# engyasin/EKF-MonoSLAM_for_3D-reconstruction

Measured on AMD Instinct MI355X. Metric: EKF updates/sec at N features (state dim 14+6N), higher is better.
Workload: dtype f32 (state, covariance, every accumulation and every other contraction in fp32; the products of the covariance downdate as 3 x bf16 splits of the fp32 operands, six bf16 products per fp32 product: the dropped terms are <= 2^-24 |a||b| in the worst case (2^-28 on average) -- the size of the fp32 prod; 1 GPU; N=1000 inverse-depth features, n=6014, M=N measured per frame, fp32, 1xMI355X (BASELINE configs[2]); features=1000, state_dim=6014, measured_per_frame=1000, camera=conf_kinect.cfg/scale2, frames_per_map=3000, maps=1

## Files before the change

ekf-monoslam_for_3d-reconstruction_amd/csrc/ekf_capi.hip:

```cpp
#include <hip/hip_runtime.h>

#include <algorithm>
#include <array>
#include <climits>
#include <cmath>
#include <cstdint>
#include <cstdio>
#include <cstdlib>
#include <cstring>
#include <map>
#include <mutex>
#include <string>
#include <type_traits>
#include <vector>

#include "../../include/ekf_monoslam.h"
#include "ekf_buffers.hpp"
#include "ekf_feature_table.hpp"
#include "ekf_dense.hpp"
#include "ekf_image.hpp"
#include "ekf_features.hpp"
#include "ekf_syrk6.hpp"
#include "ekf_chain.hpp"
#include "ekf_small.hpp"
// ... 15 lines not shown
#include "ekf_mesh_texture.hpp"
#include "ekf_mesh_raster.hpp"

namespace ekf {

static thread_local std::string g_create_error;

enum KernelId : int {
  KID_PREDICT_CAMERA = 0,
  KID_PROPAGATE_STRIPS,
  KID_PROPAGATE_STREAMING,
  KID_MEASURE,
  KID_INNOVATION,
  KID_SIGMA_HT,
  KID_INNOVATION_COV,
  KID_CHOL_DIAG,
  KID_CHOL_PANEL,
  KID_CHOL_TRAILING,
  KID_STATE_UPDATE,
  KID_DOWNDATE,
  KID_SOLVE,
  KID_NORMALIZE,
  KID_ADD_FEATURE,
  KID_COMPACT,
  KID_MISC,
  KID_WUPDATE,
  KID_GATHER_H,
  KID_GATHER_S,
  KID_GATHER_V,
  KID_GATHER_SIGMA,
  KID_SEED_MASK,
  KID_SEED_RESPONSE,
  KID_SEED_CANDIDATES,
  KID_SEED_SELECT,
  KID_FRAME_UPLOAD,
  KID_FRAME_INGEST,
  KID_FRAME_RECTIFY,
  KID_COUNT
};

static const char* kKernelNames[KID_COUNT] = {
    "predict_camera",  "propagate_strips", "propagate_streaming", "measure",
    "innovation",      "sigma_ht",         "innovation_cov",      "chol_diag",
    "chol_panel",      "chol_trailing",    "state_update",        "downdate_syrk",
    "solve_trmm",      "normalize_quat",  "add_feature",      "compact_transform",   "misc",
    "w_update", "allgather_h", "allgather_s", "allgather_v", "allgather_sigma",
    "seed_mask", "seed_response", "seed_candidates", "seed_select", "frame_upload", "frame_ingest", "frame_rectify"};

static const char* kLaunchNames[EKF_LAUNCH_KINDS] = {
    "downdate_bf16x6", "downdate_f32", "downdate_f32_fused_wu", "downdate_f32_half_tail", "downdate_f32_t64",
    "row_rider", "row_gemv", "row_tile_gemm", "w_update_gemm", "w_recompute",
    "chain_step_launches", "chain_persistent", "solve", "solve_two_groups", "update_oneblock", "update_allinone",
    "chain_trail_diag", "split_image", "state_update_tail", "update_onelaunch", "chain_dist_gather", "chain_step_fused",
    "downdate_mirror_bounds", "solve_poll_chain"};

static inline int round_up(int v, int a) { return (v + a - 1) / a * a; }

struct MaskedStreamPool {
  struct Entry { int device, num_cus, reserved; hipStream_t st; };
  std::mutex mu;
  std::vector<Entry> idle;
  bool hooked = false;
  static void at_exit();
  hipStream_t take(int device, int num_cus, int reserved) {
    std::lock_guard<std::mutex> lk(mu);
    for (size_t i = 0; i < idle.size(); ++i)
      if (idle[i].device == device && idle[i].num_cus == num_cus && idle[i].reserved == reserved) {
        hipStream_t st = idle[i].st;
        idle.erase(idle.begin() + i);
        return st;
      }
    return nullptr;
  }
  void give(int device, int num_cus, int reserved, hipStream_t st) {
    std::lock_guard<std::mutex> lk(mu);
    idle.push_back({device, num_cus, reserved, st});
    if (!hooked) { hooked = true; atexit(&MaskedStreamPool::at_exit); }
  }
};
static MaskedStreamPool g_masked_streams;
void MaskedStreamPool::at_exit() {
  std::lock_guard<std::mutex> lk(g_masked_streams.mu);
  for (const Entry& e : g_masked_streams.idle) {
    if (hipSetDevice(e.device) != hipSuccess) continue;
    (void)hipStreamSynchronize(e.st);
    (void)hipStreamDestroy(e.st);
  }
  g_masked_streams.idle.clear();
}

struct FilterBase {
  std::string err;
  bool diag_synced = false;
  virtual ~FilterBase() {}
  virtual int set_dt(double) = 0;
  virtual double get_dt() const = 0;
  virtual int set_stream(void*) = 0;
  virtual int set_option(int, int) = 0;
  virtual int synchronize() = 0;
  virtual int add_feature(double, double) = 0;
  virtual int remove_features(const int*, int) = 0;
  virtual int predict(const void*, const void*, int) = 0;
  virtual int measure() = 0;
  virtual int motion_jacobian(void*, void*) = 0;
  virtual int get_predictions(void*, unsigned char*, unsigned char*, void*, void*, void*) = 0;
  virtual int update(const void*, const int*, int, int, bool) = 0;
  virtual int innovation_covariance(const int*, int, int, void*) = 0;
// ... 114 lines not shown
  DevBuf<T> d_K;
  int last_m = 0, last_m_pad = 0, last_n = 0;
  bool have_meas = false;
  bool have_sd = false;
  bool have_update = false;
  int opt_streaming = 0, opt_mfma = 1;
  hipStream_t stream = nullptr;
  bool own_stream = false;
  hipStream_t stream_b = nullptr;
  hipEvent_t ev_chain[8] = {}, ev_solve[8] = {}, ev_b = nullptr, ev_wu = nullptr;
  hipStream_t stream_g = nullptr;
  bool stream_b_masked = false;
  int stream_b_reserved = 0;
  hipEvent_t ev_gath[8] = {}, ev_g = nullptr;
  int solve64_off = 0, solve6464_off = 0, tri64_off = 0, tri64_count = 0;
  int tri6_off = 0;
  int trih_off = 0, trih_count = 0;
  int opt_split_tail = -1;
  double opt_feature_noise = 0.0;
  int opt_split_bf16 = 1;
  DevBuf<s6_u32x4> d_Vimg;
  hipError_t ensure_vimg() { return d_Vimg.reserve((size_t)(n_pad + 128) * ldy * 6 / sizeof(s6_u32x4)); }
  int last_nchunks = 1, last_cend[8] = {};
  DevBuf<unsigned char> d_frame;
  int frame_w = 0, frame_h = 0;
  bool have_frame = false, have_blur = false;
  DevBuf<unsigned char> d_raw;
  int raw_w = 0, raw_h = 0, raw_c = 0;
  bool have_raw = false;
  RectScratch rect;
  DevBuf<int4> d_ingest_tab;
  int ingest_tab_w = 0, ingest_tab_h = 0;
  DevBuf<unsigned char> d_patch[2], d_mpatch[2];
  int cur_patch = 0;
  DevBuf<T> d_hb, d_zm;
  DevBuf<unsigned char> d_found;
  DevBuf<float> d_score;
  DevBuf<int> d_keep;
  int opt_panel_direct = 1;
  int opt_chain_fused_diag = 1;
  int opt_small_onelaunch = 1;
  int opt_step_fused = 1;
  struct StepPlan { std::vector<int> off, cnt; } sfp;
  WorkList sf_lists{{0}, {}};
  DevBuf<unsigned long long> d_small_stamps;
  unsigned small_gate_total = 0;
  int opt_su_tail = 1;
  int opt_syrk_mirror_skip = 1;
  int opt_solve_poll_chain = 1;
  int opt_fuse_split = 1;
  int opt_chain_defer = 1;
  int td_min_blocks = 24;
  int td_max_blocks = 1 << 30;
  WorkList td_blocks;
  std::vector<int> td_off, td_cnt;
  int opt_syrk_stag_half = 0, opt_syrk_stag_mod4 = 2;
  int opt_solve_s2 = 1;
  bool want_solve_s2(int width, int npad_live) const {
    return kIsF32 && opt_mfma && opt_solve_s2 && (opt_solve_s2 > 1 || (width / 128) * (npad_live / 64) <= 2 * num_cus);
  }
  int opt_fused = 1;
  int opt_solve_one_per_cu = 1;
  int opt_wrecompute = 1;
  int opt_row_gemv = 1;
  int opt_fuse_wu = 1;
  int env_chunks[8] = {}, env_nchunks = 0;
  int opt_pipeline = -1;
  WorkList tilemap{{0, 0}, {}};
  int tri_count = 0, solve_off = 0;
  int w_zeroed_n = -1;
  DevBuf<int> d_counters;
  int num_cus = 256, reserved_cus = 32;
  LaunchProfiler<KID_COUNT> prof{KID_DOWNDATE, KID_PROPAGATE_STREAMING};

  static constexpr bool kIsF32 = sizeof(T) == 4;
  int NB() const { return (kIsF32 && opt_mfma) ? 128 : 64; }

  ~Filter() override {
    const bool dbg = getenv("EKF_DEBUG_DTOR") != nullptr;
    auto mark = [&](const char* what) { if (dbg) { fprintf(stderr, "[ekf dtor %p] %s\n", (void*)this, what); fflush(stderr); } };
    hipSetDevice(device);
    mark("sync main stream");
    if (stream) hipStreamSynchronize(stream);
    mark("sync side streams");
    if (stream_b) hipStreamSynchronize(stream_b);
    if (stream_g) hipStreamSynchronize(stream_g);
    mark("events");
    prof.release();
    in_ring.release();
    mark("streams");
    if (own_stream && stream) hipStreamDestroy(stream);
    mark("stream b");
    const char* pool_env = getenv("EKF_MASKED_STREAM_POOL");
    if (stream_b && stream_b_masked && !(pool_env && atoi(pool_env) == 0)) g_masked_streams.give(device, num_cus, stream_b_reserved, stream_b);
    else if (stream_b) hipStreamDestroy(stream_b);
    mark("stream g");
    if (stream_g) hipStreamDestroy(stream_g);
    mark("last events");
    for (auto e : ev_gath) if (e) hipEventDestroy(e);
    if (ev_g) hipEventDestroy(ev_g);
    for (auto e : ev_chain) if (e) hipEventDestroy(e);
    for (auto e : ev_solve) if (e) hipEventDestroy(e);
    if (ev_b) hipEventDestroy(ev_b);
    if (ev_wu) hipEventDestroy(ev_wu);
    mark("done");
  }
// ... 71 lines not shown
    HIPCHK(d_tmp.reserve(64));
    HIPCHK(d_counters.reserve(kResetInts + kMirrorRowsInts));
    HIPCHK(hipMemset(d_counters, 0, (kResetInts + kMirrorRowsInts) * sizeof(int)));
    {
      hipDeviceProp_t prop;
      HIPCHK(hipGetDeviceProperties(&prop, device));
      num_cus = prop.multiProcessorCount > 0 ? prop.multiProcessorCount : 256;
    }
    {
      reserved_cus = std::min(32, num_cus / 4);
      if (const char* e = getenv("EKF_RESERVED_CUS")) reserved_cus = std::max(1, std::min(num_cus / 2, atoi(e)));
      std::vector<uint32_t> mask((num_cus + 31) / 32, 0xffffffffu);
      for (int i = 0; i < reserved_cus; ++i) mask[i / 32] &= ~(1u << (i % 32));
      stream_b = g_masked_streams.take(device, num_cus, reserved_cus);
      stream_b_masked = stream_b != nullptr;
      if (!stream_b) {
        if (hipExtStreamCreateWithCUMask(&stream_b, (uint32_t)mask.size(), mask.data()) == hipSuccess) {
          stream_b_masked = true;
        } else {
          (void)hipGetLastError();
          stream_b = nullptr;
          reserved_cus = 0;
          HIPCHK(hipStreamCreateWithFlags(&stream_b, hipStreamNonBlocking));
        }
      }
      stream_b_reserved = reserved_cus;

      if (const char* e = getenv("EKF_FUSE_WU")) opt_fuse_wu = atoi(e);
      if (const char* e = getenv("EKF_ROW_GEMV")) opt_row_gemv = atoi(e) ? 1 : 0;
      if (const char* e = getenv("EKF_SOLVE_ONE_PER_CU")) opt_solve_one_per_cu = atoi(e) ? 1 : 0;
      if (const char* e = getenv("EKF_W_RECOMPUTE")) opt_wrecompute = atoi(e) ? 1 : 0;
      if (const char* e = getenv("EKF_SOLVE_S2")) opt_solve_s2 = atoi(e);
      if (const char* e = getenv("EKF_FUSED_LAUNCHES")) opt_fused = atoi(e) ? 1 : 0;
      if (const char* e = getenv("EKF_PANEL_DIRECT")) opt_panel_direct = atoi(e);
      if (const char* e = getenv("EKF_SYRK_STAGGER")) {
        opt_syrk_stag_half = atoi(e);
        if (const char* c = strchr(e, ',')) opt_syrk_stag_mod4 = atoi(c + 1);
      }
      if (const char* e = getenv("EKF_CHAIN_FUSED_DIAG")) opt_chain_fused_diag = atoi(e) ? 1 : 0;
      if (const char* e = getenv("EKF_FUSE_SPLIT")) opt_fuse_split = atoi(e) ? 1 : 0;
      if (const char* e = getenv("EKF_SU_TAIL")) opt_su_tail = atoi(e) ? 1 : 0;
      if (const char* e = getenv("EKF_SYRK_MIRROR_SKIP")) opt_syrk_mirror_skip = atoi(e) ? 1 : 0;
      if (const char* e = getenv("EKF_SOLVE_POLL_CHAIN")) opt_solve_poll_chain = std::max(0, std::min(2, atoi(e)));
      if (const char* e = getenv("EKF_SMALL_ONELAUNCH")) opt_small_onelaunch = atoi(e) ? 1 : 0;
      if (const char* e = getenv("EKF_STEP_FUSED")) opt_step_fused = atoi(e) ? 1 : 0;
      if (const char* e = getenv("EKF_SHARD_DIST_CHAIN")) opt_shard_dist_chain = atoi(e) ? 1 : 0;
      if (const char* e = getenv("EKF_SHARD_DIST_MIN_BLOCKS")) shard_dist_min_blocks = std::max(2, atoi(e));
      if (const char* e = getenv("EKF_SMALL_STAMPS")) {
        if (atoi(e)) { HIPCHK(d_small_stamps.reserve(16)); HIPCHK(hipMemset(d_small_stamps, 0, 16 * sizeof(unsigned long long))); }
      }
      if (const char* e = getenv("EKF_CHAIN_DEFER")) opt_chain_defer = atoi(e) ? 1 : 0;
      if (const char* e = getenv("EKF_TD_MIN_BLOCKS")) td_min_blocks = std::max(1, atoi(e));
      if (const char* e = getenv("EKF_TD_MAX_BLOCKS")) td_max_blocks = std::max(1, atoi(e));
      if (const char* e = getenv("EKF_SPLIT_TAIL")) opt_split_tail = atoi(e);
      if (const char* e = getenv("EKF_SPLIT_BF16")) opt_split_bf16 = atoi(e) ? 1 : 0;
      if (const char* e = getenv("EKF_CHUNKS")) {
        for (const char* q = e; *q && env_nchunks < 8;) {
          env_chunks[env_nchunks++] = atoi(q);
          while (*q && *q != ',') ++q;
          if (*q == ',') ++q;
        }
      }
    }
    std::vector<T> mu0(camera_dim, T(0));
    mu0[3] = T(0.0); mu0[4] = T(0.0); mu0[5] = T(-0.707106781); mu0[6] = T(0.707106781);
    if (camera_dim == 14) mu0[13] = T(1);
    n = camera_dim;
    N = 0;
    HIPCHK(hipMemcpyAsync(d_mu[0], mu0.data(), camera_dim * sizeof(T), hipMemcpyHostToDevice, stream));
    std::vector<T> S0((size_t)camera_dim * camera_dim, T(0));
    for (int i = 0; i < camera_dim; ++i) S0[(size_t)i * camera_dim + i] = T(0.0000000004);
    if (camera_dim == 14) S0[13 * 14 + 13] = T(0.09);
    const T sv2 = T(0.0004) * T(0.0004);
    for (int i = 7; i < 13; ++i) S0[(size_t)i * camera_dim + i] = sv2;
    HIPCHK(hipMemcpy2DAsync(d_S[0], (size_t)ld * sizeof(T), S0.data(), camera_dim * sizeof(T),
                            camera_dim * sizeof(T), camera_dim, hipMemcpyHostToDevice, stream));
    HIPCHK(hipStreamSynchronize(stream));
    extent[0] = n; extent[1] = 0;
    HIPCHK(hipFuncSetAttribute(reinterpret_cast<const void*>(&k_chol_diag<T, 64>),
                               hipFuncAttributeMaxDynamicSharedMemorySize, diag_lds(64)));
    if constexpr (kIsF32) {
      HIPCHK(hipFuncSetAttribute(reinterpret_cast<const void*>(&k_trail_diag),
                                 hipFuncAttributeMaxDynamicSharedMemorySize, (int)kChainLds));
    }
    return EKF_OK;
  }
  static int diag_lds(int nb) { return 2 * nb * (nb + 1) * (int)sizeof(T); }

  T* S() { return d_S[cur]; }
  T* mu() { return d_mu[cur_mu]; }

  int sync_layout() {
    if (!layout_dirty) return EKF_OK;
    if (N > 0) {
      HIPCHK(hipMemcpyAsync(d_pos, ft.columns().pos.data(), N * sizeof(int), hipMemcpyHostToDevice, stream));
      HIPCHK(hipMemcpyAsync(d_coding, ft.columns().coding.data(), N * sizeof(int), hipMemcpyHostToDevice, stream));
      HIPCHK(hipStreamSynchronize(stream));
    }
    layout_dirty = false;
    return EKF_OK;
  }

  InputRing in_ring;
  PinnedBuf<char> h_pred;
  PinnedBuf<unsigned char> h_ransac;
  static constexpr size_t kRansacMaskBytes = 65536;
// ... 745 lines not shown
    HIPCHK(hipStreamSynchronize(stream));
    if (h) memcpy(h, ph, (size_t)N * 2 * sizeof(T));
    for (int i = 0; i < N; ++i) { if (vis) vis[i] = pfl[i] & 1; if (rem) rem[i] = (pfl[i] >> 1) & 1; }
    if (s2) {
      T* o = static_cast<T*>(s2);
      const T* sd = psd;
      for (int i = 0; i < N; ++i) { o[4 * i] = sd[4 * i]; o[4 * i + 1] = sd[4 * i + 2]; o[4 * i + 2] = sd[4 * i + 1]; o[4 * i + 3] = sd[4 * i + 3]; }
    }
    if (hc) { T* o = static_cast<T*>(hc); for (int i = 0; i < N; ++i) for (int a = 0; a < 2; ++a) for (int c = 0; c < 7; ++c) o[14 * i + c * 2 + a] = vhc[14 * i + a * 7 + c]; }
    if (hf) { T* o = static_cast<T*>(hf); for (int i = 0; i < N; ++i) for (int a = 0; a < 2; ++a) for (int c = 0; c < 6; ++c) o[12 * i + c * 2 + a] = vhf[12 * i + a * 6 + c]; }
    return EKF_OK;
  }

  struct GemmCall {
    const T* A = nullptr; int lda = 0;
    const T* B = nullptr; int ldb = 0;
    T* C = nullptr; int ldc = 0;
    int rows = 0, cols = 0, K = 0;
    T alpha = T(1), beta = T(0);
    int tri = TRI_ALL, row_off = 0, col_off = 0, ktri = KTRI_FULL, ktile_off = 0;
    int zrow = 0, zcol_end = 0;
    const int* tile_list = nullptr; int ntiles = 0;
    int* counter = nullptr;
    void* img = nullptr; int img_nkc = 0, img_c0 = 0;
    bool two_groups = false;
    bool one_per_cu = false;
    const unsigned* chain_word = nullptr; unsigned chain_epoch = 0;
    hipStream_t st = nullptr;
  };
  struct Rows { int r0, count; };
  struct UpdatePlan {
    int M = 0, plane = 0;
    int nb = 0, tile = 0, m = 0, m_pad = 0, npad_live = 0, nsteps = 0;
    int nchunks = 1, cend[8] = {};
    ChunkTab tab{};
    int strip_rows = 0;
    int ntr = 0, ntc = 0;
    bool oneblock = false, allinone = false, onelaunch = false;
    int small_rc = 0, small_nchunk = 0, small_nt64 = 0;
    bool recompute = false;
    int r0 = 0, r1 = 0, p0 = 0, prows = 0;
    Rows ranges[3] = {};
    bool sym_panel = false, shard_split = false;
    int c0(int g) const { return (g ? cend[g - 1] : 0) * nb; }
    int c1(int g) const { return cend[g] * nb; }
  };
  struct UpdateCtx {
    const T* z;
    const int* midx;
    int* counters;
    int counter_next = 0;
    bool step_fused = false;
    int diag_ahead = -1;
    struct { int step = -1, c0 = 0, c1 = 0; } pending;
    bool row_pending = false;
    bool queue_room(int ints = 8) const { return counter_next + ints <= kQueueCounters; }
    int* take_queue() {
      if (!queue_room()) return nullptr;
      counter_next += 8;
      return counters + counter_next - 8;
    }
  };

  template <int ROLE, bool BT, int TM = 128, int TN = 128>
  void gemm(const GemmCall& c) {
    GemmArgs g{};
    g.A = c.A; g.lda = c.lda; g.B = c.B; g.ldb = c.ldb; g.C = c.C; g.ldc = c.ldc;
    g.K = c.K; g.alpha = double(c.alpha); g.beta = double(c.beta);
    g.tri = c.tri; g.row_off = c.row_off; g.col_off = c.col_off; g.ktri = c.ktri; g.ktile_off = c.ktile_off;
    g.zrow = c.zrow; g.zcol_end = c.zcol_end;
    g.stagger = (ROLE == ROLE_DOWNDATE) ? 1 : 0;
    g.img = c.img; g.img_nkc = c.img_nkc; g.img_c0 = c.img_c0;
    g.chain_word = c.chain_word; g.chain_epoch = c.chain_epoch; g.status = d_status;
    hipStream_t st = c.st ? c.st : stream;
    const bool mf = kIsF32 && opt_mfma;
    dim3 grid(c.cols / (mf ? TN : 64), c.rows / (mf ? TM : 64));
    if (c.tile_list && c.counter) {
      g.tile_map = c.tile_list;
      g.ntiles = c.ntiles;
      g.counter = c.counter;
      const bool side = (st == stream_b);
      int wgs = 2 * (side ? (num_cus - reserved_cus) : num_cus);
      if (ROLE == ROLE_SOLVE && c.one_per_cu) wgs = num_cus;
      grid = dim3(std::min(c.ntiles, wgs), 1);
    }
    if constexpr (kIsF32) {
      if (opt_mfma) {
        if constexpr (ROLE == ROLE_SOLVE) {
          ++launch_cnt[c.two_groups ? EKF_LAUNCH_SOLVE_TWO_GROUPS : EKF_LAUNCH_SOLVE];
          if (c.two_groups) {
            k_gemm_mfma<ROLE, BT, TM, TN, true><<<grid, 512, 0, st>>>(g);
            return;
          }
        }
        k_gemm_mfma<ROLE, BT, TM, TN><<<grid, 256, 0, st>>>(g);
        return;
      }
    }
    if constexpr (!kIsF32) {
      if (opt_mfma) {
        k_gemm_mfma_f64<ROLE, BT><<<grid, 256, 0, st>>>(g);
        return;
      }
    }
    k_gemm_valu<T, ROLE, BT><<<grid, 256, 0, st>>>(g);
  }
// ... 174 lines not shown
        constexpr int KB = 8;
        dim3 grid((m_pad + 255) / 256, std::max(1, (M + KB - 1) / KB) + (m_pad - 2 * M + 7) / 8);
        k_innovation_cov<T, KB><<<grid, 256, 0, stream>>>(d_W, ldy, d_Hc, d_Hf, d_pos, d_coding, ip, M, plane,
                                                        T(sigma_pixel_2), T(0.00001), d_Y, m_pad, 0, M, zid, N, ct, strip_rows);
      }
    }
    HIPCHK(hipGetLastError());
    if (m_out) *m_out = m;
    if (m_pad_out) *m_pad_out = m_pad;
    return EKF_OK;
  }

  bool trail_diag_ok() const {
    return kIsF32 && opt_mfma && opt_chain_fused_diag && (size_t)2 * ldy * ldy * sizeof(T) < ((size_t)1 << 31);
  }
  int ensure_trail_diag_lists(int nblk, int nchunks, const int* cend) {
    std::vector<int> key = {nblk, nchunks};
    key.insert(key.end(), cend, cend + nchunks);
    if (td_blocks.current(key)) return EKF_OK;
    std::vector<int> all;
    td_off.assign(nblk, 0);
    td_cnt.assign(nblk, 0);
    for (int g = 0; g < nchunks; ++g) {
      const int s0 = g ? cend[g - 1] : 0, s1 = cend[g];
      for (int j = s0; j < s1; ++j) {
        td_off[j] = (int)all.size();
        for (int K = j + 1; K < nblk; ++K) {
          for (int I = K; I < nblk; ++I) {
            if (I == j + 1) continue;
            all.push_back(I); all.push_back(K);
          }
          if (K < s1)
            for (int t = 0; t <= j - s0; ++t) { all.push_back(nblk + t); all.push_back(K); }
        }
        td_cnt[j] = ((int)all.size() - td_off[j]) / 2;
      }
    }
    HIPCHK(hipStreamSynchronize(stream));
    if (stream_b) HIPCHK(hipStreamSynchronize(stream_b));
    HIPCHK(td_blocks.upload(key, all, 2));
    return EKF_OK;
  }
  bool launch_trail_diag(UpdateCtx& ux, int step, int m, hipStream_t sc_) {
    if constexpr (kIsF32) {
      const int td_nblk = td_blocks.first();
      if (!trail_diag_ok() || NB() != 128 || td_nblk == 0 || step + 1 >= td_nblk || td_cnt[step] < td_min_blocks ||
          td_cnt[step] > td_max_blocks)
        return false;
      TrailDiagArgs a{};
      a.Y = d_Y; a.ldy = ldy; a.y_bytes = (unsigned)((size_t)2 * ldy * ldy * sizeof(T));
      a.Dinv = d_Dinv; a.dinv_bytes = (unsigned)((size_t)(ldy / 64) * 128 * 128 * sizeof(T));
      a.status = d_status; a.m = m; a.j = step;
      a.blocks = td_blocks.d + td_off[step]; a.nblocks = td_cnt[step]; a.do_diag = 1;
      Scope sc(this, KID_CHOL_TRAILING, sc_);
      ++launch_cnt[EKF_LAUNCH_CHAIN_TRAIL_DIAG];
      k_trail_diag<<<a.nblocks + 1, 1024, kChainLds, sc_>>>(a);
      ux.diag_ahead = step + 1;
      return true;
    }
    return false;
  }

  int ensure_step_fused_lists(int nblk) {
    const std::vector<int> key = {nblk};
    if (sf_lists.current(key)) return EKF_OK;
    std::vector<int> all;
    sfp.off.assign(nblk, 0);
    sfp.cnt.assign(nblk, 0);
    const int s0 = 0, s1 = nblk;
    for (int j = 0; j < nblk; ++j) {
      sfp.off[j] = (int)all.size();
      const int first = 2 * (j + 1);
      for (int r = first; r < 2 * nblk; ++r)
        for (int c = first; c <= r; ++c) { all.push_back(r); all.push_back(c); all.push_back(SF_TILE | (c == r ? SF_WRITE_PANEL : 0)); }
      for (int r = 2 * nblk; r < 2 * nblk + 2 * (j + 1 - s0); ++r) {
        if (first < 2 * s1) {
          for (int c = first; c < 2 * s1; ++c) { all.push_back(r); all.push_back(c); all.push_back(SF_TILE | (c == first ? SF_WRITE_PANEL : 0)); }
        } else {
          all.push_back(r); all.push_back(r); all.push_back(SF_WRITE_PANEL);
        }
      }
      sfp.cnt[j] = ((int)all.size() - sfp.off[j]) / 3;
      all[sfp.off[j] + 2] |= SF_WRITE_DIAG;
    }
    HIPCHK(hipStreamSynchronize(stream));
    HIPCHK(sf_lists.upload(key, all));
    return EKF_OK;
  }
  bool launch_step_fused(const UpdateCtx& ux, int step, int m, hipStream_t sc_) {
    if constexpr (kIsF32) {
      if (!ux.step_fused || step >= sf_lists.first() || sfp.cnt[step] > num_cus / 2 || sc_ != stream) return false;
      StepFusedArgs a{};
      a.Y = d_Y; a.ldy = ldy; a.Dj = d_Dinv + (size_t)step * 128 * 128; a.status = d_status; a.m = m; a.j = step;
      a.wl = sf_lists.d + sfp.off[step]; a.nwg = sfp.cnt[step];
      a.gate = reinterpret_cast<unsigned*>(d_status + 9);
      small_gate_total += (unsigned)a.nwg;
      a.gate_target = small_gate_total;
      Scope sc(this, KID_CHOL_TRAILING, sc_);
      ++launch_cnt[EKF_LAUNCH_CHAIN_STEP_FUSED];
      k_chain_step_fused<<<a.nwg, 1024, 0, sc_>>>(a);
      return true;
    }
    return false;
  }
  void chain_trailing(UpdateCtx& ux, int step, int c0, int c1, int m, int m_pad, hipStream_t sc_, bool allow_fused) {
    const int nb = NB();
    T* Y = d_Y;
    const int j = step * nb, r0 = j + nb;
    const int vrows = m_pad - c0, tcols = m_pad - r0;
// ... 407 lines not shown
        std::vector<int> hidx((size_t)std::max(M, 0));
        if (M > 0) {
          HIPCHK(hipMemcpyAsync(hidx.data(), idx, (size_t)M * sizeof(int), hipMemcpyDeviceToHost, stream));
          HIPCHK(hipStreamSynchronize(stream));
        }
        return shard_update(z, hidx.data(), M, plane);
      }
      if (M > 0 && z) HIPCHK(hipMemcpyAsync(d_z, z, (size_t)2 * M * sizeof(T), hipMemcpyHostToDevice, stream));
      return shard_update(d_z, idx, M, plane);
    }
    if (M < 0 || M > N) FAIL(EKF_ERR_ARG, "M out of range");
    if (M == 0 && !plane) return EKF_OK;
    if (!have_meas) FAIL(EKF_ERR_STATE, "ekf_update needs the h/H of ekf_predict or ekf_measure");
    if (M > 0 && (!z || !idx)) FAIL(EKF_ERR_ARG, "z / indices are NULL");
    if (!on_device) { int rcl = check_list(idx, M, true); if (rcl) return rcl; }
    UpdateCtx ux{d_z, d_midx, d_counters};
    if (M > 0) {
      if (on_device) {
        ux.z = static_cast<const T*>(z);
        ux.midx = idx;
      } else {
        int rcs = stage_inputs(z, idx, M);
        if (rcs) return rcs;
        sh_list.clear();
      }
    }
    const UpdatePlan p = plan_update(M, plane);
    int rc = p.onelaunch ? launch_update_small(p, ux)
                         : build_innovation(ux.z, ux.midx, M, plane, true, nullptr, nullptr, &p.tab, p.strip_rows);
    if (rc) return rc;
    rc = ensure_tilemap(p.npad_live / p.tile, p.ntr, p.ntc);
    if (rc) return rc;
    rc = prepare_chain(p, ux, false);
    if (rc) return rc;
    const int nchunks = p.nchunks, m_pad = p.m_pad;
    bool b_inflight = false;
    for (int gi = 0; gi < (p.onelaunch ? 0 : nchunks); ++gi) {
      const int c0 = p.c0(gi), c1 = p.c1(gi);
      chain_steps(ux, gi ? p.cend[gi - 1] : 0, p.cend[gi], c0, c1, p.m, m_pad, stream, p.oneblock,
                  opt_chain_defer && gi + 1 < nchunks);
      const bool overlap = chunk_overlaps(p, gi);
      hipStream_t ss = overlap ? stream_b : stream;
      if (!overlap && b_inflight) {
        if (p.recompute) {
          HIPCHK(hipEventRecord(ev_b, stream_b));
          HIPCHK(hipStreamWaitEvent(stream, ev_b, 0));
          b_inflight = false;
        } else {
          HIPCHK(hipStreamWaitEvent(stream, ev_wu, 0));
        }
      }
      if (overlap) {
        b_inflight = true;
        if (solve_polls_chain(p, gi)) {
          if constexpr (kIsF32)
            k_publish_epoch<<<1, 64, 0, stream>>>(reinterpret_cast<unsigned*>(d_counters + kChainEpochWord), (unsigned)gi + 1);
        } else {
          HIPCHK(hipEventRecord(ev_chain[gi], stream));
          HIPCHK(hipStreamWaitEvent(stream_b, ev_chain[gi], 0));
        }
      }
      bool vimg_done = false;
      rc = solve_chunk(p, gi, ux, ss, &vimg_done);
      if (rc) return rc;
      const bool fuse = chunk_fuses(p, gi, ux);
      wupdate_chunk(p, gi, ux, ss);
      if (overlap && c1 < m_pad && !fuse && !p.recompute) HIPCHK(hipEventRecord(ev_wu, stream_b));
      if (!overlap && b_inflight) {
        HIPCHK(hipEventRecord(ev_b, stream_b));
        HIPCHK(hipStreamWaitEvent(stream, ev_b, 0));
        b_inflight = false;
      }
      if (!overlap && nchunks > 1 && !chunk_su_tail(p, gi, ux)) {
        HIPCHK(hipEventRecord(ev_chain[gi], stream));
        HIPCHK(hipStreamWaitEvent(stream_b, ev_chain[gi], 0));
        launch_state_update(m_pad, stream_b);
        b_inflight = true;
      }
      rc = downdate_chunk(p, gi, ux, ss, vimg_done);
      if (rc) return rc;
      if (fuse && !p.recompute) HIPCHK(hipEventRecord(ev_wu, stream_b));
      if (p.recompute && gi + 1 < nchunks) {
        launch_w_recompute(c1, p.c1(gi + 1), m_pad, ux.midx, M, plane, ss, n);
      }
    }
    if (b_inflight) {
      HIPCHK(hipEventRecord(ev_b, stream_b));
      HIPCHK(hipStreamWaitEvent(stream, ev_b, 0));
    }
    return finish_update(p, nchunks == 1 && !p.oneblock, !p.allinone);
  }

  int innovation_covariance(const int* idx, int M, int plane, void* out) override {
    HIPCHK(hipSetDevice(device));
    if (M < 0 || M > N) FAIL(EKF_ERR_ARG, "M out of range");
    if (!have_meas) FAIL(EKF_ERR_STATE, "ekf_innovation_covariance needs ekf_predict / ekf_measure first");
    const int mm = 2 * M + (plane ? 3 : 0);
    if (mm == 0) return EKF_OK;
    int rc = check_list(idx, M, sh_on);
    if (rc) return rc;
    if (M > 0) HIPCHK(hipMemcpyAsync(d_midx, idx, (size_t)M * sizeof(int), hipMemcpyHostToDevice, stream));
    sh_list.clear();
    int m = 0, m_pad = 0;
    if (sh_on) {
      rc = shard_build_ws(idx, M, plane, nullptr, &m, &m_pad);
    } else {
// ... 4266 lines not shown
```

ekf-monoslam_for_3d-reconstruction_amd/csrc/ekf_chain.hpp:

```cpp
#pragma once
#include "ekf_dense.hpp"

namespace ekf {

constexpr unsigned kChainPimg = 75776;
constexpr unsigned kChainLds = 141568;

namespace chain {
typedef float f4 __attribute__((ext_vector_type(4)));
typedef __amdgpu_buffer_rsrc_t rsrc_t;

__device__ __forceinline__ f4 ld16(rsrc_t r, unsigned byte_off) {
  return __builtin_bit_cast(f4, __builtin_amdgcn_raw_buffer_load_b128(r, (int)byte_off, 0, 0));
}
__device__ __forceinline__ float ld4(rsrc_t r, unsigned byte_off) {
  return __builtin_bit_cast(float, __builtin_amdgcn_raw_buffer_load_b32(r, (int)byte_off, 0, 0));
}
__device__ __forceinline__ void st4(rsrc_t r, unsigned byte_off, float v) {
  __builtin_amdgcn_raw_buffer_store_b32(__builtin_bit_cast(unsigned, v), r, (int)byte_off, 0, 0);
}

__device__ __attribute__((noinline)) void trail(rsrc_t ry, unsigned ldy, int j, int I, int K, int only, f32x4* lds_all, int tid,
                                                int lane, int wave) {
  constexpr int NQ = 8, TS = 64, STAGE = NQ * (TS + TS), BK = 32, NG = BK / 8;
  const int grp = wave >> 2, gr = grp >> 1, gc = grp & 1;
  const bool active = !(I == K && gr == 0 && gc == 1) && (only < 0 || only == grp);
  f32x4* lds = lds_all + grp * 2 * STAGE;
  const int t = tid & 255, w4 = wave & 3, wr = w4 >> 1, wc = w4 & 1;
  const int h = lane >> 5, l31 = lane & 31;
  const int arow0 = I * 128 + gr * 64, brow0 = K * 128 + gc * 64, kcol0 = j * 128;
  unsigned aoff[2], boff[2];
  int aslot[2], bslot[2];
#pragma unroll
  for (int p = 0; p < 2; ++p) {
    const int idx = t + 256 * p;
    const int row = idx >> 3, q = idx & 7;
    aoff[p] = (((unsigned)(arow0 + row)) * ldy + (unsigned)(kcol0 + q * 4)) * 4u;
    boff[p] = (((unsigned)(brow0 + row)) * ldy + (unsigned)(kcol0 + q * 4)) * 4u;
    aslot[p] = q * TS + (row ^ q);
    bslot[p] = q * TS + (row ^ q);
  }
  f32x16 acc;
#pragma unroll
  for (int e = 0; e < 16; ++e) acc[e] = 0.f;
  f4 ra[2], rb[2];
  auto load_tile = [&](int k0) {
#pragma unroll
    for (int p = 0; p < 2; ++p) { ra[p] = ld16(ry, aoff[p] + 4u * k0); rb[p] = ld16(ry, boff[p] + 4u * k0); }
  };
  auto store_tile = [&](int stage) {
    f32x4* As = lds + stage * STAGE;
    f32x4* Bs = As + NQ * TS;
#pragma unroll
    for (int p = 0; p < 2; ++p) { As[aslot[p]] = ra[p]; Bs[bslot[p]] = rb[p]; }
  };
  f32x4 fa[2], fb[2];
  auto read_frag = [&](int stage, int s, int buf) {
    const f32x4* As = lds + stage * STAGE;
    const f32x4* Bs = As + NQ * TS;
    const int q = 2 * s + h;
    fa[buf] = As[q * TS + ((wr * 32 + l31) ^ q)];
    fb[buf] = Bs[q * TS + ((wc * 32 + l31) ^ q)];
  };
  auto mfma_group = [&](int buf) {
#pragma unroll
    for (int e = 0; e < 4; ++e) acc = __builtin_amdgcn_mfma_f32_32x32x2f32(fa[buf][e], fb[buf][e], acc, 0, 0, 0);
  };
  if (active) { load_tile(0); store_tile(0); load_tile(BK); }
  __syncthreads();
  if (active) read_frag(0, 0, 0);
  int stage = 0;
#pragma unroll
  for (int ks = 0; ks < 4; ++ks) {
    const bool more = ks < 3, more2 = ks < 2;
#pragma unroll
    for (int s = 0; s < NG; ++s) {
      if (s + 1 < NG) {
        if (active) read_frag(stage, s + 1, (s + 1) & 1);
      } else {
        __syncthreads();
        if (active && more) read_frag(stage ^ 1, 0, 0);
      }
      if (active) mfma_group(s & 1);
      if (s == 0 && more && active) {
        store_tile(stage ^ 1);
        if (more2) load_tile(BK * (ks + 2));
      }
    }
    stage ^= 1;
  }
  if (!active) return;
  const unsigned c = (unsigned)(brow0 + wc * 32 + l31);
  const unsigned rbase = (unsigned)(arow0 + wr * 32 + 4 * h);
  float v[16];
#pragma unroll
  for (int e = 0; e < 16; ++e) v[e] = 1.f * ld4(ry, ((rbase + (e & 3) + 8 * (e >> 2)) * ldy + c) * 4u);
#pragma unroll
  for (int e = 0; e < 16; ++e) v[e] = __builtin_fmaf(-1.f, acc[e], v[e]);
#pragma unroll
  for (int e = 0; e < 16; ++e) st4(ry, ((rbase + (e & 3) + 8 * (e >> 2)) * ldy + c) * 4u, v[e]);
}

__device__ __forceinline__ void load_diag_c(rsrc_t ry, unsigned ldy, int blk, int wave, int lane, float (&cv)[16]) {
  const int h = lane >> 5, l31 = lane & 31;
  const int bi = wave >= 6 ? 3 : (wave >= 3 ? 2 : (wave >= 1 ? 1 : 0)), bj = wave - bi * (bi + 1) / 2;
  if (wave < 10) {
    const unsigned c = (unsigned)(blk * 128 + 32 * bj + l31), r0 = (unsigned)(blk * 128 + 32 * bi + 4 * h);
#pragma unroll
    for (int e = 0; e < 16; ++e) cv[e] = ld4(ry, ((r0 + (e & 3) + 8 * (e >> 2)) * ldy + c) * 4u);
  }
}
__device__ __forceinline__ void update_diag_image(const f32x4* pimg, float* a, int wave, int lane, const float (&cv)[16]) {
  constexpr int LDA = 132;
  const int h = lane >> 5, l31 = lane & 31;
  if (wave < 10) {
    const int bi = wave >= 6 ? 3 : (wave >= 3 ? 2 : (wave >= 1 ? 1 : 0)), bj = wave - bi * (bi + 1) / 2;
    f32x16 acc;
#pragma unroll
    for (int e = 0; e < 16; ++e) acc[e] = 0.f;
#pragma unroll
    for (int ks = 0; ks < 4; ++ks)
#pragma unroll
      for (int sg = 0; sg < 4; ++sg) {
        const int q = 2 * sg + h, kq = ks * 8 + q;
        const f32x4 fa = pimg[kq * 128 + ((32 * bi + l31) ^ q)];
        const f32x4 fb = pimg[kq * 128 + ((32 * bj + l31) ^ q)];
#pragma unroll
        for (int e = 0; e < 4; ++e) acc = __builtin_amdgcn_mfma_f32_32x32x2f32(fa[e], fb[e], acc, 0, 0, 0);
      }
#pragma unroll
    for (int e = 0; e < 16; ++e) {
      const int row = 32 * bi + (e & 3) + 8 * (e >> 2) + 4 * h, col = 32 * bj + l31;
      const float v = __builtin_fmaf(-1.f, acc[e], 1.f * cv[e]);
      a[row * LDA + col] = (col <= row) ? v : 0.f;
    }
  } else {
    const int u = wave - 10;
    const int zi = u < 3 ? 0 : (u < 5 ? 1 : 2), zj = u < 3 ? u + 1 : (u < 5 ? u - 1 : 3);
#pragma unroll
    for (int r = 0; r < 16; ++r) a[(32 * zi + 16 * h + r) * LDA + 32 * zj + l31] = 0.f;
  }
}
}

struct TrailDiagArgs {
  float* Y; int ldy; unsigned y_bytes;
  float* Dinv; unsigned dinv_bytes;
  int* status;
  int m;
  int j;
  const int* blocks; int nblocks;
  int do_diag;
};

__global__ void __launch_bounds__(1024) k_trail_diag(TrailDiagArgs g) {
  using namespace chain;
  extern __shared__ __attribute__((aligned(16))) unsigned char chain_smem[];
  const int tid = threadIdx.x;
  const int lane = tid & 63, wave = __builtin_amdgcn_readfirstlane(tid >> 6);
  const rsrc_t ry = __builtin_amdgcn_make_buffer_rsrc(g.Y, 0, (int)g.y_bytes, 0x27000);
  const unsigned ldy = (unsigned)g.ldy;
  __builtin_amdgcn_s_setprio(2);
  if (g.do_diag && blockIdx.x == 0) {
    const int j = g.j, blk = g.j + 1;
    float* a = reinterpret_cast<float*>(chain_smem);
    f32x4* pimg = reinterpret_cast<f32x4*>(chain_smem + kChainPimg);
    f4 v[4];
#pragma unroll
    for (int p = 0; p < 4; ++p) {
      const int idx = tid + 1024 * p, row = idx >> 5, kq = idx & 31;
      v[p] = ld16(ry, (((unsigned)(blk * 128 + row)) * ldy + (unsigned)(j * 128 + 4 * kq)) * 4u);
    }
    float cv[16];
    load_diag_c(ry, ldy, blk, wave, lane, cv);
#pragma unroll
    for (int p = 0; p < 4; ++p) {
      const int idx = tid + 1024 * p, row = idx >> 5, kq = idx & 31;
      pimg[kq * 128 + (row ^ (kq & 7))] = v[p];
    }
    __syncthreads();
    update_diag_image(pimg, a, wave, lane, cv);
    const DiagLds L{a, reinterpret_cast<float(*)[16 * 20]>(a + 128 * 132),
                    reinterpret_cast<float(*)[16]>(a + 128 * 132 + 2 * 16 * 20), a + 128 * 132 + 2 * 16 * 20 + 2 * 16};
    diag_factor_lds<7>(g.status, max(1, min(8, (g.m - blk * 128 + 15) / 16)), L);
    float* Ab = g.Y + (size_t)blk * 128 * g.ldy + (size_t)blk * 128;
    float* Db = g.Dinv + (size_t)blk * 128 * 128;
    const int ld_ = g.ldy;
    diag_store_lds([&](int i, int j0, const f4& x) { *reinterpret_cast<f4*>(Ab + (size_t)i * ld_ + j0) = x; },
                   [&](int i, int jj, float x) { Db[(size_t)i * 128 + jj] = x; }, a);
    return;
  }
  const int t = (int)blockIdx.x - g.do_diag;
  if (t >= g.nblocks) return;
  const int I = g.blocks[2 * t], K = g.blocks[2 * t + 1];
  trail(ry, ldy, g.j, I, K, -1, reinterpret_cast<f32x4*>(chain_smem), tid, lane, wave);
}

}
```

include/ekf_monoslam.h:

```cpp
#ifndef EKF_MONOSLAM_H_
#define EKF_MONOSLAM_H_

#include <stddef.h>

#ifdef __cplusplus
extern "C" {
#endif

#define EKF_ABI_VERSION 6

typedef struct ekf_filter ekf_filter;

enum ekf_dtype { EKF_F32 = 0, EKF_F64 = 1 };

enum ekf_status {
  EKF_OK = 0,
  EKF_ERR_ARG = 1,
  EKF_ERR_CAPACITY = 2,
  EKF_ERR_DEVICE = 3,
  EKF_ERR_STATE = 4,
  EKF_ERR_NUMERIC = 5,
  EKF_ERR_UNSUPPORTED = 6
};

// ... 88 lines not shown
int ekf_get_sigma_block(ekf_filter* f, void* out, int r0, int c0, int rows, int cols);
int ekf_set_sigma_block(ekf_filter* f, const void* in, int r0, int c0, int rows, int cols);
int ekf_peek_workspace(ekf_filter* f, int which, void* out, int r0, int c0, int rows, int cols);
int ekf_covariance_parameter(ekf_filter* f, double* out);
int ekf_check_invariants(ekf_filter* f, double* max_abs_outside_live, double* max_asymmetry, double* max_abs_live);
int ekf_feature_xyz(ekf_filter* f, int index, void* xyz, void* cov3x3);

int ekf_export_points(ekf_filter* f, void* out, int convert_inverse_depth);
int ekf_export_points_table(ekf_filter* f, void* out, int max_rows, int* rows);
int ekf_get_feature_ids(const ekf_filter* f, int* real_index, int* n_find);
int ekf_set_feature_meta(ekf_filter* f, int index, int real_index, int n_find);
int ekf_num_archived(const ekf_filter* f);

int ekf_get_feature_track(ekf_filter* f, int* n_tot, unsigned char* in_innovation, float* center,
                          unsigned char* remove_flag);
int ekf_set_feature_track(ekf_filter* f, int index, int n_tot, int in_innovation, const float* center, int remove_flag);
int ekf_find_new_features(ekf_filter* f, int num, double quality_level, double min_distance, int add, float* out_uv,
                          int* n_out);
int ekf_end_update(ekf_filter* f, float matching_ratio, int seed, int* removed, int* n_removed, int* n_visible,
                   int* n_seeded);

int ekf_profile_kernels(void);
const char* ekf_profile_kernel_name(int kernel_id);
int ekf_profile_read(ekf_filter* f, int kernel_id, double* total_ms, long long* launches);
int ekf_profile_reset(ekf_filter* f);
int ekf_profile_work(ekf_filter* f, int kernel_id, double* flop);
int ekf_get_chunk_plan(ekf_filter* f, int* ends, int max_chunks, int* block, int* w_recompute);

enum ekf_launch_kind {
  EKF_LAUNCH_DOWNDATE_BF16X6 = 0,
  EKF_LAUNCH_DOWNDATE_F32,
  EKF_LAUNCH_DOWNDATE_F32_FUSED_WU,
  EKF_LAUNCH_DOWNDATE_F32_HALF_TAIL,
  EKF_LAUNCH_DOWNDATE_F32_T64,
  EKF_LAUNCH_ROW_RIDER,
  EKF_LAUNCH_ROW_GEMV,
  EKF_LAUNCH_ROW_TILE_GEMM,
  EKF_LAUNCH_W_UPDATE_GEMM,
  EKF_LAUNCH_W_RECOMPUTE,
  EKF_LAUNCH_CHAIN_STEP,
  EKF_LAUNCH_CHAIN_PERSISTENT,
  EKF_LAUNCH_SOLVE,
  EKF_LAUNCH_SOLVE_TWO_GROUPS,
  EKF_LAUNCH_UPDATE_ONEBLOCK,
  EKF_LAUNCH_UPDATE_ALLINONE,
  EKF_LAUNCH_CHAIN_TRAIL_DIAG,
  EKF_LAUNCH_SPLIT_IMAGE,
  EKF_LAUNCH_STATE_UPDATE_TAIL,
  EKF_LAUNCH_UPDATE_ONELAUNCH,
  EKF_LAUNCH_CHAIN_DIST_GATHER,
  EKF_LAUNCH_CHAIN_STEP_FUSED,
  EKF_LAUNCH_DOWNDATE_MIRROR_BOUNDS,
  EKF_LAUNCH_SOLVE_POLL_CHAIN,
  EKF_LAUNCH_KINDS
};
int ekf_launch_kinds(void);
const char* ekf_launch_kind_name(int kind);
int ekf_launch_count(ekf_filter* f, int kind, long long* launches);

typedef int (*ekf_allgather_fn)(void* ctx, const void* d_send, void* d_recv, size_t bytes_per_rank, void* hip_stream);

typedef struct ekf_shard_info {
  int rank, world, N, state_dim;
  int f_begin, f_end;
  int row_begin, row_end;
  int max_rows_any_rank;
  int rebalances;
} ekf_shard_info;

int ekf_shard_configure(ekf_filter* f, int rank, int world, ekf_allgather_fn allgather, void* ctx);
int ekf_shard_get_info(ekf_filter* f, ekf_shard_info* out);
int ekf_shard_update(ekf_filter* f, const void* d_z, const int* indices, int M, int plane_constraint);
int ekf_shard_rebalance(ekf_filter* f);

void* ekf_device_mu(ekf_filter* f);
void* ekf_device_sigma(ekf_filter* f, int* ld);

#define EKF_SBA_SOLVER_CHOLESKY 0
#define EKF_SBA_SOLVER_BPCG 3

typedef struct ekf_sba ekf_sba;
typedef struct ekf_sba_camera {
  double fx, fy, cx, cy;
} ekf_sba_camera;

int ekf_sba_create(const ekf_sba_camera* K, int capacity_nodes, int capacity_points, int capacity_projections,
                   int device, ekf_sba** out);
int ekf_sba_create_solver(const ekf_sba_camera* K, int capacity_nodes, int capacity_points, int capacity_projections,
                          int device, int solver, ekf_sba** out);
int ekf_sba_get_solver(const ekf_sba* s, int* solver);
int ekf_sba_set_cg(ekf_sba* s, double init_tol, int max_iters);
int ekf_sba_get_cg(const ekf_sba* s, double* init_tol, int* max_iters);
int ekf_sba_get_cg_log(const ekf_sba* s, int max_rows, int* cg_iters, double* dn_final, double* d0, int* n);
void ekf_sba_destroy(ekf_sba* s);
const char* ekf_sba_last_error(const ekf_sba* s);
int ekf_sba_add_nodes(ekf_sba* s, int n, const double* pose7);
int ekf_sba_add_points(ekf_sba* s, int n, const double* xyz);
int ekf_sba_add_projections(ekf_sba* s, int n, const int* node, const int* point, const double* uv, int* added);
int ekf_sba_counts(const ekf_sba* s, int* nodes, int* points, int* projections);
int ekf_sba_run(ekf_sba* s, int niter, double lambda, int* iterations);
int ekf_sba_cost(ekf_sba* s, double dist, double* sq_cost, double* rms);
int ekf_sba_set_huber(ekf_sba* s, double huber);
int ekf_sba_get_huber(const ekf_sba* s, double* huber);
int ekf_sba_count_bad(ekf_sba* s, double dist, int* n);
int ekf_sba_remove_bad(ekf_sba* s, double dist, int* n);
int ekf_sba_reduce_tracks(ekf_sba* s, int* cleared);
// ... 175 lines not shown
```

Baseline: 1132 updates/s.

## Pack Cholesky trailing tiles into persistent workgroups with cross-tile prefetch

Rewrites the trailing-update kernel so each workgroup loops over several 128x128 tiles with a grid stride, prefetching the next tile's first K-slices and the C values during the current tile's MFMA loop. The grid can be capped via EKF_TD_PACK_WGS, and when overlapped with a masked solve stream the cap can follow the reserved CU count (pack value -1). The aim is fewer idle workgroups and better overlap of loads with compute when the chain shares the GPU with the solve. With default td_pack_wgs=0 the grid is unchanged, but the new loop structure and the early C load still run.

```diff
diff --git a/ekf-monoslam_for_3d-reconstruction_amd/csrc/ekf_capi.hip b/ekf-monoslam_for_3d-reconstruction_amd/csrc/ekf_capi.hip
--- a/ekf-monoslam_for_3d-reconstruction_amd/csrc/ekf_capi.hip
+++ b/ekf-monoslam_for_3d-reconstruction_amd/csrc/ekf_capi.hip
@@ -91,7 +91,7 @@
     "row_rider", "row_gemv", "row_tile_gemm", "w_update_gemm", "w_recompute",
     "chain_step_launches", "chain_persistent", "solve", "solve_two_groups", "update_oneblock", "update_allinone",
     "chain_trail_diag", "split_image", "state_update_tail", "update_onelaunch", "chain_dist_gather", "chain_step_fused",
-    "downdate_mirror_bounds", "solve_poll_chain"};
+    "downdate_mirror_bounds", "solve_poll_chain", "chain_trail_packed"};
 
 static inline int round_up(int v, int a) { return (v + a - 1) / a * a; }
 
@@ -312,6 +312,7 @@
   int opt_chain_defer = 1;
   int td_min_blocks = 24;
   int td_max_blocks = 1 << 30;
+  int td_pack_wgs = 0;
   WorkList td_blocks;
   std::vector<int> td_off, td_cnt;
   int opt_syrk_stag_half = 0, opt_syrk_stag_mod4 = 2;
@@ -489,6 +490,7 @@
       if (const char* e = getenv("EKF_CHAIN_DEFER")) opt_chain_defer = atoi(e) ? 1 : 0;
       if (const char* e = getenv("EKF_TD_MIN_BLOCKS")) td_min_blocks = std::max(1, atoi(e));
       if (const char* e = getenv("EKF_TD_MAX_BLOCKS")) td_max_blocks = std::max(1, atoi(e));
+      if (const char* e = getenv("EKF_TD_PACK_WGS")) td_pack_wgs = std::max(-1, atoi(e));
       if (const char* e = getenv("EKF_SPLIT_TAIL")) opt_split_tail = atoi(e);
       if (const char* e = getenv("EKF_SPLIT_BF16")) opt_split_bf16 = atoi(e) ? 1 : 0;
       if (const char* e = getenv("EKF_CHUNKS")) {
@@ -1340,6 +1342,7 @@
     int counter_next = 0;
     bool step_fused = false;
     int diag_ahead = -1;
+    int td_pack_cap = 0;
     struct { int step = -1, c0 = 0, c1 = 0; } pending;
     bool row_pending = false;
     bool queue_room(int ints = 8) const { return counter_next + ints <= kQueueCounters; }
@@ -1620,9 +1623,12 @@
       a.Dinv = d_Dinv; a.dinv_bytes = (unsigned)((size_t)(ldy / 64) * 128 * 128 * sizeof(T));
       a.status = d_status; a.m = m; a.j = step;
       a.blocks = td_blocks.d + td_off[step]; a.nblocks = td_cnt[step]; a.do_diag = 1;
+      const int cap = td_pack_wgs < 0 ? ux.td_pack_cap : (sh_on ? 0 : td_pack_wgs);
+      const int wgs = cap > 0 ? std::min(a.nblocks, cap) : a.nblocks;
       Scope sc(this, KID_CHOL_TRAILING, sc_);
       ++launch_cnt[EKF_LAUNCH_CHAIN_TRAIL_DIAG];
-      k_trail_diag<<<a.nblocks + 1, 1024, kChainLds, sc_>>>(a);
+      if (wgs < a.nblocks) ++launch_cnt[EKF_LAUNCH_CHAIN_TRAIL_PACKED];
+      k_trail_diag<<<wgs + 1, 1024, kChainLds, sc_>>>(a);
       ux.diag_ahead = step + 1;
       return true;
     }
@@ -2136,6 +2142,7 @@
       }
       if (overlap) {
         b_inflight = true;
+        if (stream_b_masked && reserved_cus > 1) ux.td_pack_cap = reserved_cus - 1;
         if (solve_polls_chain(p, gi)) {
           if constexpr (kIsF32)
             k_publish_epoch<<<1, 64, 0, stream>>>(reinterpret_cast<unsigned*>(d_counters + kChainEpochWord), (unsigned)gi + 1);
diff --git a/ekf-monoslam_for_3d-reconstruction_amd/csrc/ekf_chain.hpp b/ekf-monoslam_for_3d-reconstruction_amd/csrc/ekf_chain.hpp
--- a/ekf-monoslam_for_3d-reconstruction_amd/csrc/ekf_chain.hpp
+++ b/ekf-monoslam_for_3d-reconstruction_amd/csrc/ekf_chain.hpp
@@ -20,39 +20,37 @@
   __builtin_amdgcn_raw_buffer_store_b32(__builtin_bit_cast(unsigned, v), r, (int)byte_off, 0, 0);
 }
 
-__device__ __attribute__((noinline)) void trail(rsrc_t ry, unsigned ldy, int j, int I, int K, int only, f32x4* lds_all, int tid,
-                                                int lane, int wave) {
+__device__ __forceinline__ void trail_blocks(rsrc_t ry, unsigned ldy, int j, const int* blocks, int t0, int nblocks, int stride,
+                                             f32x4* lds_all, int tid, int lane, int wave) {
   constexpr int NQ = 8, TS = 64, STAGE = NQ * (TS + TS), BK = 32, NG = BK / 8;
   const int grp = wave >> 2, gr = grp >> 1, gc = grp & 1;
-  const bool active = !(I == K && gr == 0 && gc == 1) && (only < 0 || only == grp);
   f32x4* lds = lds_all + grp * 2 * STAGE;
   const int t = tid & 255, w4 = wave & 3, wr = w4 >> 1, wc = w4 & 1;
   const int h = lane >> 5, l31 = lane & 31;
-  const int arow0 = I * 128 + gr * 64, brow0 = K * 128 + gc * 64, kcol0 = j * 128;
-  unsigned aoff[2], boff[2];
-  int aslot[2], bslot[2];
+  const int kcol0 = j * 128;
+  unsigned roff[2];
+  int slot[2];
 #pragma unroll
   for (int p = 0; p < 2; ++p) {
     const int idx = t + 256 * p;
     const int row = idx >> 3, q = idx & 7;
-    aoff[p] = (((unsigned)(arow0 + row)) * ldy + (unsigned)(kcol0 + q * 4)) * 4u;
-    boff[p] = (((unsigned)(brow0 + row)) * ldy + (unsigned)(kcol0 + q * 4)) * 4u;
-    aslot[p] = q * TS + (row ^ q);
-    bslot[p] = q * TS + (row ^ q);
+    roff[p] = (((unsigned)row) * ldy + (unsigned)(kcol0 + q * 4)) * 4u;
+    slot[p] = q * TS + (row ^ q);
   }
   f32x16 acc;
-#pragma unroll
-  for (int e = 0; e < 16; ++e) acc[e] = 0.f;
   f4 ra[2], rb[2];
-  auto load_tile = [&](int k0) {
-#pragma unroll
-    for (int p = 0; p < 2; ++p) { ra[p] = ld16(ry, aoff[p] + 4u * k0); rb[p] = ld16(ry, boff[p] + 4u * k0); }
+  auto load_tile = [&](int arow0, int brow0, int k0) {
+#pragma unroll
+    for (int p = 0; p < 2; ++p) {
+      ra[p] = ld16(ry, (unsigned)arow0 * ldy * 4u + roff[p] + 4u * k0);
+      rb[p] = ld16(ry, (unsigned)brow0 * ldy * 4u + roff[p] + 4u * k0);
+    }
   };
   auto store_tile = [&](int stage) {
     f32x4* As = lds + stage * STAGE;
     f32x4* Bs = As + NQ * TS;
 #pragma unroll
-    for (int p = 0; p < 2; ++p) { As[aslot[p]] = ra[p]; Bs[bslot[p]] = rb[p]; }
+    for (int p = 0; p < 2; ++p) { As[slot[p]] = ra[p]; Bs[slot[p]] = rb[p]; }
   };
   f32x4 fa[2], fb[2];
   auto read_frag = [&](int stage, int s, int buf) {
@@ -66,39 +64,62 @@
 #pragma unroll
     for (int e = 0; e < 4; ++e) acc = __builtin_amdgcn_mfma_f32_32x32x2f32(fa[buf][e], fb[buf][e], acc, 0, 0, 0);
   };
-  if (active) { load_tile(0); store_tile(0); load_tile(BK); }
+  int I = blocks[2 * t0], K = blocks[2 * t0 + 1];
+  bool active = !(I == K && gr == 0 && gc == 1);
+  int arow0 = I * 128 + gr * 64, brow0 = K * 128 + gc * 64;
+  if (active) { load_tile(arow0, brow0, 0); store_tile(0); load_tile(arow0, brow0, BK); }
   __syncthreads();
   if (active) read_frag(0, 0, 0);
-  int stage = 0;
-#pragma unroll
-  for (int ks = 0; ks < 4; ++ks) {
-    const bool more = ks < 3, more2 = ks < 2;
-#pragma unroll
-    for (int s = 0; s < NG; ++s) {
-      if (s + 1 < NG) {
-        if (active) read_frag(stage, s + 1, (s + 1) & 1);
-      } else {
-        __syncthreads();
-        if (active && more) read_frag(stage ^ 1, 0, 0);
+  for (int tb = t0;;) {
+    const int tn = tb + stride;
+    const bool has_next = tn < nblocks;
+    const int In = has_next ? blocks[2 * tn] : I, Kn = has_next ? blocks[2 * tn + 1] : K;
+    const bool active_n = has_next && !(In == Kn && gr == 0 && gc == 1);
+    const int arow0_n = In * 128 + gr * 64, brow0_n = Kn * 128 + gc * 64;
+    const unsigned c = (unsigned)(brow0 + wc * 32 + l31);
+    const unsigned rbase = (unsigned)(arow0 + wr * 32 + 4 * h);
+    float v[16];
+#pragma unroll
+    for (int e = 0; e < 16; ++e) acc[e] = 0.f;
+#pragma unroll
+    for (int ks = 0; ks < 4; ++ks) {
+      const int stage = ks & 1;
+#pragma unroll
+      for (int s = 0; s < NG; ++s) {
+        if (s + 1 < NG) {
+          if (active) read_frag(stage, s + 1, (s + 1) & 1);
+        } else {
+          __syncthreads();
+          if (ks < 3 ? active : active_n) read_frag(stage ^ 1, 0, 0);
+        }
+        if (active) mfma_group(s & 1);
+        if (s == 0) {
+          if (ks < 3) {
+            if (active) {
+              store_tile(stage ^ 1);
+              if (ks < 2) load_tile(arow0, brow0, BK * (ks + 2));
+            }
+            if (ks == 0 && active) {
+#pragma unroll
+              for (int e = 0; e < 16; ++e) v[e] = 1.f * ld4(ry, ((rbase + (e & 3) + 8 * (e >> 2)) * ldy + c) * 4u);
+            }
+            if (ks == 2 && active_n) load_tile(arow0_n, brow0_n, 0);
+          } else if (active_n) {
+            store_tile(stage ^ 1);
+            load_tile(arow0_n, brow0_n, BK);
+          }
+        }
       }
-      if (active) mfma_group(s & 1);
-      if (s == 0 && more && active) {
-        store_tile(stage ^ 1);
-        if (more2) load_tile(BK * (ks + 2));
-      }
-    }
-    stage ^= 1;
-  }
-  if (!active) return;
-  const unsigned c = (unsigned)(brow0 + wc * 32 + l31);
-  const unsigned rbase = (unsigned)(arow0 + wr * 32 + 4 * h);
-  float v[16];
-#pragma unroll
-  for (int e = 0; e < 16; ++e) v[e] = 1.f * ld4(ry, ((rbase + (e & 3) + 8 * (e >> 2)) * ldy + c) * 4u);
-#pragma unroll
-  for (int e = 0; e < 16; ++e) v[e] = __builtin_fmaf(-1.f, acc[e], v[e]);
-#pragma unroll
-  for (int e = 0; e < 16; ++e) st4(ry, ((rbase + (e & 3) + 8 * (e >> 2)) * ldy + c) * 4u, v[e]);
+    }
+    if (active) {
+#pragma unroll
+      for (int e = 0; e < 16; ++e) v[e] = __builtin_fmaf(-1.f, acc[e], v[e]);
+#pragma unroll
+      for (int e = 0; e < 16; ++e) st4(ry, ((rbase + (e & 3) + 8 * (e >> 2)) * ldy + c) * 4u, v[e]);
+    }
+    if (!has_next) break;
+    tb = tn; I = In; K = Kn; active = active_n; arow0 = arow0_n; brow0 = brow0_n;
+  }
 }
 
 __device__ __forceinline__ void load_diag_c(rsrc_t ry, unsigned ldy, int blk, int wave, int lane, float (&cv)[16]) {
@@ -192,8 +213,7 @@
   }
   const int t = (int)blockIdx.x - g.do_diag;
   if (t >= g.nblocks) return;
-  const int I = g.blocks[2 * t], K = g.blocks[2 * t + 1];
-  trail(ry, ldy, g.j, I, K, -1, reinterpret_cast<f32x4*>(chain_smem), tid, lane, wave);
-}
-
-}
+  trail_blocks(ry, ldy, g.j, g.blocks, t, g.nblocks, (int)gridDim.x - g.do_diag, reinterpret_cast<f32x4*>(chain_smem), tid, lane, wave);
+}
+
+}
diff --git a/include/ekf_monoslam.h b/include/ekf_monoslam.h
--- a/include/ekf_monoslam.h
+++ b/include/ekf_monoslam.h
@@ -164,6 +164,7 @@
   EKF_LAUNCH_CHAIN_STEP_FUSED,
   EKF_LAUNCH_DOWNDATE_MIRROR_BOUNDS,
   EKF_LAUNCH_SOLVE_POLL_CHAIN,
+  EKF_LAUNCH_CHAIN_TRAIL_PACKED,
   EKF_LAUNCH_KINDS
 };
 int ekf_launch_kinds(void);
```

Result: no change. 1137 updates/s (median of 4 runs) (+0.5%).
